# shihchinw/rlShaders

Hardware: AMD Instinct MI355X
Metric: BSDF Gsamples/sec (eval+sample+pdf) (higher is better)
Workload: dtype f32

## Files before the change

__graft_entry__.py:

```python
from __future__ import annotations

import os
import subprocess
import sys
from pathlib import Path

ROOT = Path(__file__).resolve().parent
REF_SRC_DEFAULT = "/root/reference"
for p in (str(ROOT), str(ROOT / "tests")):
    if p not in sys.path:
        sys.path.insert(0, p)


def build() -> None:
    from rlshaders_amd import build as b
    lib = b.build_library(verbose=False)
    assert lib.exists(), lib
    b.build_host_examples()
    b.build_trace_example()
    p = subprocess.run(["make", "-C", str(ROOT / "oracle")], capture_output=True, text=True)
    if p.returncode != 0:
        raise RuntimeError(f"oracle build failed:\n{p.stdout}\n{p.stderr}")
    ref_src = Path(os.environ.get("RLS_REF_SRC", REF_SRC_DEFAULT))
    if (ref_src / "src" / "rlGgx.h").exists():
        p = subprocess.run(["make", "-C", str(ROOT / "oracle"), "ref", f"REF_SRC={ref_src}"], capture_output=True,
                           text=True)
        if p.returncode != 0:
            raise RuntimeError(f"reference build failed:\n{p.stdout}\n{p.stderr}")
    import rlshaders_amd
    rlshaders_amd.load()
    from rlshaders_amd import trace
    trace.load()


def smoke() -> None:
    import numpy as np
    import torch

    import cases
    import oracle_lib as O
    import rlshaders_amd as R
    from gpu_util import dev, ggx_oracle, ggx_sampler, host

    assert torch.cuda.is_available(), "smoke() needs a GPU"
    ctx = R.Context(0)
    n = 1 << 14
    c = cases.ggx_mixed(cases.SEED_PARITY, n)
    x = cases.xi(cases.SEED_PARITY, n, 4)
    s = ggx_sampler(ctx, c)
    out = [host(t) for t in s.reflectRefract(dev(x[0]), dev(x[1]), dev(x[2]), dev(x[3]))]
    ref = ggx_oracle(O, c).reflect_refract(x[0], x[1], x[2], x[3])
    names = ("wi", "f", "pdf", "fresnel", "wt", "weight")
    for name, a, b in zip(names, out, ref):
        st = cases.summarize(cases.rel_err(a, b))
        print(f"smoke {name}: median {st['median']:.2e} p99.9 {st['p999']:.2e} frac>1e-5 {st['frac_gt_1e5']:.2e}")
        assert st["nonfinite"] == 0 and st["max"] <= 1e-5, (name, st)
    f = host(s.evalBrdf(dev(ref[0])))
    assert cases.summarize(cases.rel_err(f, ref[1]))["max"] <= 1e-5
    ctx.close()
    print("smoke ok")


if __name__ == "__main__":
    build()
    if len(sys.argv) > 1 and sys.argv[1] == "smoke":
        smoke()
```

rlshaders_amd/build.py:

```python
from __future__ import annotations

import os
import shutil
import subprocess
import sys
from concurrent.futures import ThreadPoolExecutor
from pathlib import Path

PKG = Path(__file__).resolve().parent
CSRC = PKG / "csrc"
LIBDIR = PKG / "lib"
OBJDIR = PKG / "build"
LIB = LIBDIR / "librlshaders_amd.so"
ARCH = "gfx950"

SOURCES = ["shade.hip", "integrate.hip", "lights.hip", "scatter.hip", "skin.hip", "ggx.hip", "disney.hip", "sss.hip", "alternates.hip", "context.hip", "pipeline.hip",
           "libm_check.hip"]
FAST_UNITS = {"ggx.hip", "disney.hip", "sss.hip", "skin.hip", "integrate.hip", "lights.hip", "scatter.hip", "shade.hip", "alternates.hip"}
HEADERS = [CSRC / "rls_device.hpp", CSRC / "rls_libm.hpp", CSRC / "rls_libm_tables.inc", CSRC / "rls_libm_flavour_args.inc", CSRC / "rls_internal.hpp", CSRC / "rls_loops.hpp",
           PKG.parent / "include" / "rlshaders_amd.h", PKG.parent / "include" / "rlshaders_amd_diag.h"]

HIPCC_FLAGS = [
    f"--offload-arch={ARCH}", "-O3", "-std=c++17", "-fPIC",
    "-ffp-contract=off", "-fno-fast-math",
    "-fno-slp-vectorize",
    "-fno-gpu-rdc",
    "-Wall", "-Wno-unused-function",
]


def _hipcc() -> str:
    exe = shutil.which("hipcc") or "/opt/rocm/bin/hipcc"
    if not os.path.exists(exe):
        raise RuntimeError("hipcc not found: the rlshaders_amd HIP library cannot be built")
    return exe


def _stale(target: Path, deps) -> bool:
    if not target.exists():
        return True
    t = target.stat().st_mtime
    return any(Path(d).stat().st_mtime > t for d in deps)


def sources():
    return [CSRC / s for s in SOURCES if (CSRC / s).exists()]


def build_library(force: bool = False, verbose: bool = False, variant: str = "", defines=(), extra=()) -> Path:
    hipcc = _hipcc()
    LIBDIR.mkdir(exist_ok=True)
    objdir = OBJDIR if not variant else PKG / f"build_{variant}"
    lib = LIB if not variant else LIBDIR / f"librlshaders_amd_{variant}.so"
    objdir.mkdir(exist_ok=True)
    srcs = sources()
    jobs = []
    objs = []
    for src in srcs:
        flavours = [("", "RLS_FAST=0")] + ([("_fast", "RLS_FAST=1")] if src.name in FAST_UNITS else [])
        for suffix, flag in flavours:
            obj = objdir / (src.stem + suffix + ".o")
            objs.append(obj)
            if force or _stale(obj, [src, *HEADERS, Path(__file__)]):
                jobs.append([hipcc, *HIPCC_FLAGS, *extra, f"-cuid=rlshaders_amd.{src.stem}{suffix}", f"-D{flag}",
                             *[f"-D{d}" for d in defines], "-c", str(src), "-o", str(obj)])

    def run(cmd):
        if verbose:
            print(" ".join(cmd), flush=True)
        p = subprocess.run(cmd, capture_output=True, text=True)
        if p.returncode != 0:
            raise RuntimeError(f"hipcc failed:\n{' '.join(cmd)}\n{p.stdout}\n{p.stderr}")
        return p

    if jobs:
        with ThreadPoolExecutor(max_workers=min(4, len(jobs))) as ex:
            list(ex.map(run, jobs))
    if force or jobs or _stale(lib, objs):
        run([hipcc, f"--offload-arch={ARCH}", "-shared", "-fPIC", "-o", str(lib), *map(str, objs)])
    return lib


TRACE_CSRC = PKG / "csrc_trace"
TRACE_SOURCES = ["trace.hip"]
TRACE_LIB = LIBDIR / "librls_trace.so"
TRACE_HEADERS = [TRACE_CSRC / "rls_trace_device.hpp", PKG.parent / "include" / "rlshaders_amd_trace.h"]


def build_trace_library(force: bool = False, verbose: bool = False) -> Path:
    hipcc = _hipcc()
    main = build_library(verbose=verbose)
    objdir = OBJDIR / "trace"
    objdir.mkdir(parents=True, exist_ok=True)
    jobs, objs = [], []
    for name in TRACE_SOURCES:
        src = TRACE_CSRC / name
        for suffix, flag in (("", "RLS_FAST=0"), ("_fast", "RLS_FAST=1")):
            obj = objdir / (src.stem + suffix + ".o")
            objs.append(obj)
            if force or _stale(obj, [src, *HEADERS, *TRACE_HEADERS, Path(__file__)]):
                jobs.append([hipcc, *HIPCC_FLAGS, f"-cuid=rls_trace.{src.stem}{suffix}", f"-D{flag}", "-c", str(src),
                             "-o", str(obj)])

    def run(cmd):
        if verbose:
            print(" ".join(cmd), flush=True)
        p = subprocess.run(cmd, capture_output=True, text=True)
        if p.returncode != 0:
            raise RuntimeError(f"hipcc failed:\n{' '.join(cmd)}\n{p.stdout}\n{p.stderr}")

    if jobs:
        with ThreadPoolExecutor(max_workers=min(4, len(jobs))) as ex:
            list(ex.map(run, jobs))
    if force or jobs or _stale(TRACE_LIB, [*objs, main]):
        run([hipcc, f"--offload-arch={ARCH}", "-shared", "-fPIC", "-o", str(TRACE_LIB), *map(str, objs),
             f"-L{LIBDIR}", "-lrlshaders_amd", "-Wl,-rpath,$ORIGIN"])
    return TRACE_LIB


def build_trace_example(verbose: bool = False) -> Path:
    OBJDIR.mkdir(exist_ok=True)
    lib = build_trace_library(verbose=verbose)
    src, out = PKG / "host" / "example_trace.cpp", OBJDIR / "example_trace"
    if _stale(out, [src, PKG / "host" / "rls_trace.hpp", lib, LIB, *HEADERS, *TRACE_HEADERS]):
        cmd = ["g++", "-std=c++14", "-O2", "-Wall", f"-I{PKG.parent / 'include'}", f"-I{PKG / 'host'}", str(src), "-o", str(out),
               f"-L{LIBDIR}", "-lrls_trace", "-lrlshaders_amd", f"-Wl,-rpath,{LIBDIR}", "-L/opt/rocm/lib", "-Wl,-rpath,/opt/rocm/lib"]
        if verbose:
            print(" ".join(cmd), flush=True)
        p = subprocess.run(cmd, capture_output=True, text=True)
        if p.returncode != 0:
            raise RuntimeError(f"host example example_trace failed to build:\n{p.stdout}\n{p.stderr}")
    return out


def build_host_examples(verbose: bool = False) -> Path:
    OBJDIR.mkdir(exist_ok=True)
    first = OBJDIR / "example_arnold_stub"
    for name in ("example_arnold_stub", "example_multi_gpu", "example_host_pipeline", "test_arnold_stub"):
        src = PKG / "host" / f"{name}.cpp"
        out = OBJDIR / name
        if not src.exists():
            continue
        if _stale(out, [src, PKG / "host" / "rls_batch.hpp", PKG / "host" / "rl_arnold_stub.hpp", LIB, *HEADERS]):
            cmd = ["g++", "-std=c++14", "-O2", "-Wall", "-pthread", f"-I{PKG.parent / 'include'}", f"-I{PKG / 'host'}",
                   str(src), "-o", str(out), f"-L{LIBDIR}", "-lrlshaders_amd", f"-Wl,-rpath,{LIBDIR}",
                   "-L/opt/rocm/lib", "-Wl,-rpath,/opt/rocm/lib"]
            if verbose:
                print(" ".join(cmd), flush=True)
            p = subprocess.run(cmd, capture_output=True, text=True)
            if p.returncode != 0:
                raise RuntimeError(f"host example {name} failed to build:\n{p.stdout}\n{p.stderr}")
    return first


if __name__ == "__main__":
    args = sys.argv[1:]
    variant = args[args.index("--variant") + 1] if "--variant" in args else ""
    defines = [a[2:] for a in args if a.startswith("-D")]
    extra = []
    for i, a in enumerate(args):
        if a.startswith(("-f", "-m", "-O")):
            extra.append(a)
            if a == "-mllvm":
                extra.append(args[i + 1])
    print(build_library(force="--force" in args, verbose=True, variant=variant, defines=defines, extra=extra))
```

rlshaders_amd/csrc/ggx.hip:

```cpp
#include "rls_internal.hpp"

using namespace rlsd;

namespace {

using namespace rlsh;

#define RLS_GGX_ARGS(a0) reload_args(a0)

enum { MIXED = 0, STREAMED_ALL = 1, UNIFORM_MATERIAL = 2 };

template <int MODE>
__device__ __forceinline__ Ggx load_closure(const rls_ggx_closure &c, Idx i, const GgxMaterial &um)
{
    constexpr bool STREAMED = MODE == STREAMED_ALL;
    V3 wo = ld3(c.wo, i), N = ld3(c.N, i), T = ld3(c.T, i);
    const PIndex<Idx> k = pindex<MODE == MIXED>(c.materials, i);
    float kr, kg, kb;
    ldrgb<STREAMED>(c.KsColor, k, kr, kg, kb);
    if (MODE == UNIFORM_MATERIAL)
        return ggx_from_material(um, wo, N, T, c.exiting ? (c.exiting[i.full()] != 0) : false, kr, kg, kb);
    float rough = ldp<STREAMED>(c.specularRoughness, k);
    float ior = ldp<STREAMED>(c.ior, k);
    float aniso = ldp<STREAMED>(c.anisotropic, k);
    bool exiting = c.exiting ? (c.exiting[i.full()] != 0) : false;
    return ggx_make(wo, N, T, exiting, kr, kg, kb, ior, rough, aniso);
}

#ifndef RLS_GGX_WAVES
#define RLS_GGX_WAVES(OP) ((OP) == OP_EVAL ? 6 : 8)
#endif
#define RLS_GGX_ATTR(OP) __launch_bounds__(rlsh::kBlock) __attribute__((amdgpu_waves_per_eu(RLS_GGX_WAVES(OP), RLS_GGX_WAVES(OP))))
template <int OP, int FAST_MATH, int MODE>
__device__ __forceinline__ void ggx_body(const GgxIO &a0)
{
    if (OP == OP_SAMPLE || OP == OP_FUSED || OP == OP_REFLECT_REFRACT || OP == OP_REFRACT || OP == OP_MICROFACET)
        stage_libm_tables();
    GgxMaterial um = {};
    if (MODE == UNIFORM_MATERIAL) {
        const rls_ggx_closure &c = a0.c;
        um = ggx_material_wave_uniform(ggx_material(c.ior.u, c.specularRoughness.u, c.anisotropic.u));
    }
    const TileRange tiles = tile_range(a0.n);
    for (int64_t base = tiles.first; base < tiles.end; base += tiles.step) {
        const Idx i = make_idx(base);
        if (i.full() >= a0.n) continue;
        const GgxIO a = RLS_GGX_ARGS(a0);
        Ggx g = load_closure<MODE>(a.c, i, um);

        if (OP == OP_SAMPLE || OP == OP_FUSED || OP == OP_REFLECT_REFRACT) {
            float rx = ldg(a.rx, i), ry = ldg(a.ry, i);
            VndfView w = vndf_view(g.view, g.fr, g.ax, g.ay);
            V3 M, M2;
            if (OP == OP_REFLECT_REFRACT) {
                float rx2 = ldg(a.rx2, i), ry2 = ldg(a.ry2, i);
                vndf_microfacet_pair(w, g.fr, rx, ry, w, g.fr, rx2, ry2, M, M2);
            } else {
                M = vndf_microfacet(w, g.fr, rx, ry);
            }
            V3 L = reflect_direction(g.view, M);
            float F = ggx_fresnel(g, L, M);
            {
                const GgxIO b = RLS_GGX_ARGS(a0);
                st3(b.wi, i, L);
                if (b.fresnel) stg(b.fresnel, i, F);
            }
            if (OP != OP_SAMPLE) {
                float fr, fg, fb, pdf;
                ggx_eval_pdf<true, true>(g, L, fr, fg, fb, pdf);
                const GgxIO b = RLS_GGX_ARGS(a0);
                strgb(b.f, i, fr, fg, fb);
                stg(b.pdf, i, pdf);
            }
            if (OP == OP_REFLECT_REFRACT) {
                V3 dir;
                ggx_refract(g, M2, dir);
                const float wgt = ggx_sample_weight(g, g.view, dir, M2);
                const GgxIO b = RLS_GGX_ARGS(a0);
                st3(b.wt, i, dir);
                stg(b.weight, i, wgt);
            }
        } else if (OP == OP_EVAL) {
            float fr, fg, fb;
            ggx_eval(g, ld3(a.cwi, i), fr, fg, fb);
            strgb(a.f, i, fr, fg, fb);
        } else if (OP == OP_PDF) {
            stg(a.pdf, i, ggx_pdf(g, ld3(a.cwi, i)));
        } else if (OP == OP_REFRACT) {
            float rx = ldg(a.rx, i), ry = ldg(a.ry, i);
            VndfView w = vndf_view(g.view, g.fr, g.ax, g.ay);
            V3 M = vndf_microfacet(w, g.fr, rx, ry);
            V3 dir;
            bool ok = ggx_refract(g, M, dir);
            st3(a.wt, i, dir);
            stg(a.weight, i, ggx_sample_weight(g, g.view, dir, M));
            if (a.refracted) a.refracted[i.full()] = ok ? 1 : 0;
        } else if (OP == OP_MICROFACET) {
            float rx = ldg(a.rx, i), ry = ldg(a.ry, i);
            V3 M;
            if (a.kernel == RLS_KERNEL_NDF) {
                M = ndf_microfacet(g, rx, ry);
            } else {
                VndfView w = vndf_view(g.view, g.fr, g.ax, g.ay);
                M = vndf_microfacet(w, g.fr, rx, ry);
            }
            st3(a.wi, i, M);
        } else if (OP == OP_NDF_PDF) {
            V3 H = normalize(g.view + ld3(a.cwi, i));
            stg(a.pdf, i, ndf_pdf(g, g.view, H));
        }
    }
}

template <int OP, int FAST_MATH, int MODE>
__global__ RLS_GGX_ATTR(OP) void ggx_kernel(GgxIO a0)
{
    ggx_body<OP, FAST_MATH, MODE>(a0);
}

#if RLS_DIAGNOSTICS
template <int OP, int FAST_MATH, int MODE>
__global__ RLS_GGX_ATTR(OP) void ggx_kernel_stamped(GgxIO a0, unsigned long long *stamps)
{
    ClockStamp<1> cs;
    cs.begin();
    ggx_body<OP, FAST_MATH, MODE>(a0);
    cs.end(stamps);
}
#endif

template <int OP>
rls_status launch_kernel(rls_context *ctx, const GgxIO &io, const char *name)
{
    const rls_ggx_closure &c = io.c;
    const bool streamed = !c.materials.id && c.KsColor.r && c.specularRoughness.v && c.ior.v && c.anisotropic.v;
    const bool uniform = !c.materials.id && !c.specularRoughness.v && !c.ior.v && !c.anisotropic.v;
    if constexpr (OP == OP_REFLECT_REFRACT)
        RLS_STAMPED_LAUNCH(streamed, (ggx_kernel_stamped<OP, RLS_FAST, STREAMED_ALL>),
                           rlsh::grid_for(ctx, io.n, rlsh::kBlock, RLS_CAP_MULT), io, name);
    if (streamed)
        hipLaunchKernelGGL((ggx_kernel<OP, RLS_FAST, STREAMED_ALL>), rlsh::grid_for(ctx, io.n, rlsh::kBlock, RLS_CAP_MULT), dim3(rlsh::kBlock), 0, ctx->stream, io);
    else if (uniform)
        hipLaunchKernelGGL((ggx_kernel<OP, RLS_FAST, UNIFORM_MATERIAL>), rlsh::grid_for_hoisting(ctx, io.n), dim3(rlsh::kBlock), 0, ctx->stream, io);
    else
        hipLaunchKernelGGL((ggx_kernel<OP, RLS_FAST, MIXED>), rlsh::grid_for(ctx, io.n, rlsh::kBlock, RLS_CAP_MULT), dim3(rlsh::kBlock), 0, ctx->stream, io);
    return rlsh::check_launch(name, RLS_FAST);
}

rls_status launch_ggx(rls_context *ctx, int op, const GgxIO &io, const char *name)
{
    switch (op) {
    case OP_SAMPLE: return launch_kernel<OP_SAMPLE>(ctx, io, name);
    case OP_EVAL: return launch_kernel<OP_EVAL>(ctx, io, name);
    case OP_PDF: return launch_kernel<OP_PDF>(ctx, io, name);
    case OP_FUSED: return launch_kernel<OP_FUSED>(ctx, io, name);
    case OP_REFRACT: return launch_kernel<OP_REFRACT>(ctx, io, name);
    case OP_REFLECT_REFRACT: return launch_kernel<OP_REFLECT_REFRACT>(ctx, io, name);
    case OP_MICROFACET: return launch_kernel<OP_MICROFACET>(ctx, io, name);
    default: return launch_kernel<OP_NDF_PDF>(ctx, io, name);
    }
}

}

RLS_FLAVOURS(ggx, rlsh::GgxIO)

#if !RLS_FAST

extern "C" {

rls_status rls_ggx_sample(rls_context *ctx, int64_t n, const rls_ggx_closure *c,
                          const float *rx, const float *ry, rls_vec3 wi, float *fresnel)
{
    RLS_PROLOGUE();
    if (rls_status s = rlsh::check_closure(__func__, c)) return s;
    RLS_REQUIRE(rx && ry, "rx/ry is NULL");
    RLS_REQUIRE(rlsh::has3(wi), "wi plane is NULL");
    GgxIO io = {};
    io.c = *c; io.rx = rx; io.ry = ry; io.wi = wi; io.fresnel = fresnel; io.n = n;
    return dispatch_ggx(ctx, OP_SAMPLE, io, "rls_ggx_sample");
}

rls_status rls_ggx_eval(rls_context *ctx, int64_t n, const rls_ggx_closure *c, rls_cvec3 wi, rls_rgb f)
{
    RLS_PROLOGUE();
    if (rls_status s = rlsh::check_closure(__func__, c)) return s;
    RLS_REQUIRE(rlsh::has3(wi) && rlsh::has3(f), "wi/f plane is NULL");
    GgxIO io = {};
    io.c = *c; io.cwi = wi; io.f = f; io.n = n;
    return dispatch_ggx(ctx, OP_EVAL, io, "rls_ggx_eval");
}

rls_status rls_ggx_pdf(rls_context *ctx, int64_t n, const rls_ggx_closure *c, rls_cvec3 wi, float *pdf)
{
    RLS_PROLOGUE();
    if (rls_status s = rlsh::check_closure(__func__, c)) return s;
    RLS_REQUIRE(rlsh::has3(wi) && pdf, "wi/pdf is NULL");
    GgxIO io = {};
    io.c = *c; io.cwi = wi; io.pdf = pdf; io.n = n;
    return dispatch_ggx(ctx, OP_PDF, io, "rls_ggx_pdf");
}

rls_status rls_ggx_sample_eval_pdf(rls_context *ctx, int64_t n, const rls_ggx_closure *c,
                                   const float *rx, const float *ry,
                                   rls_vec3 wi, rls_rgb f, float *pdf, float *fresnel)
{
    RLS_PROLOGUE();
    if (rls_status s = rlsh::check_closure(__func__, c)) return s;
    RLS_REQUIRE(rx && ry, "rx/ry is NULL");
    RLS_REQUIRE(rlsh::has3(wi) && rlsh::has3(f) && pdf, "wi/f/pdf is NULL");
    GgxIO io = {};
    io.c = *c; io.rx = rx; io.ry = ry; io.wi = wi; io.f = f; io.pdf = pdf; io.fresnel = fresnel; io.n = n;
    return dispatch_ggx(ctx, OP_FUSED, io, "rls_ggx_sample_eval_pdf");
}

rls_status rls_ggx_refract_sample(rls_context *ctx, int64_t n, const rls_ggx_closure *c,
                                  const float *rx, const float *ry,
                                  rls_vec3 wt, float *weight, uint8_t *refracted)
{
    RLS_PROLOGUE();
    if (rls_status s = rlsh::check_closure(__func__, c)) return s;
    RLS_REQUIRE(rx && ry, "rx/ry is NULL");
    RLS_REQUIRE(rlsh::has3(wt) && weight, "wt/weight is NULL");
    GgxIO io = {};
    io.c = *c; io.rx = rx; io.ry = ry; io.wt = wt; io.weight = weight; io.refracted = refracted; io.n = n;
    return dispatch_ggx(ctx, OP_REFRACT, io, "rls_ggx_refract_sample");
}

rls_status rls_ggx_reflect_refract(rls_context *ctx, int64_t n, const rls_ggx_closure *c,
                                   const float *rx, const float *ry, const float *rx2, const float *ry2,
                                   rls_vec3 wi, rls_rgb f, float *pdf, float *fresnel,
                                   rls_vec3 wt, float *weight)
{
    RLS_PROLOGUE();
    if (rls_status s = rlsh::check_closure(__func__, c)) return s;
    RLS_REQUIRE(rx && ry && rx2 && ry2, "random-number plane is NULL");
    RLS_REQUIRE(rlsh::has3(wi) && rlsh::has3(f) && pdf, "wi/f/pdf is NULL");
    RLS_REQUIRE(rlsh::has3(wt) && weight, "wt/weight is NULL");
    GgxIO io = {};
    io.c = *c; io.rx = rx; io.ry = ry; io.rx2 = rx2; io.ry2 = ry2;
    io.wi = wi; io.f = f; io.pdf = pdf; io.fresnel = fresnel; io.wt = wt; io.weight = weight; io.n = n;
    return dispatch_ggx(ctx, OP_REFLECT_REFRACT, io, "rls_ggx_reflect_refract");
}

rls_status rls_ggx_microfacet(rls_context *ctx, int64_t n, const rls_ggx_closure *c, int kernel,
                              const float *rx, const float *ry, rls_vec3 m)
{
    RLS_PROLOGUE();
    if (rls_status s = rlsh::check_closure(__func__, c)) return s;
    RLS_REQUIRE(kernel == RLS_KERNEL_VNDF || kernel == RLS_KERNEL_NDF, "unknown sampling kernel");
    RLS_REQUIRE(rx && ry, "rx/ry is NULL");
    RLS_REQUIRE(rlsh::has3(m), "m plane is NULL");
    GgxIO io = {};
    io.c = *c; io.rx = rx; io.ry = ry; io.wi = m; io.kernel = kernel; io.n = n;
    return dispatch_ggx(ctx, OP_MICROFACET, io, "rls_ggx_microfacet");
}

rls_status rls_ggx_ndf_pdf(rls_context *ctx, int64_t n, const rls_ggx_closure *c, rls_cvec3 wi, float *pdf)
{
    RLS_PROLOGUE();
    if (rls_status s = rlsh::check_closure(__func__, c)) return s;
    RLS_REQUIRE(rlsh::has3(wi) && pdf, "wi/pdf is NULL");
    GgxIO io = {};
    io.c = *c; io.cwi = wi; io.pdf = pdf; io.n = n;
    return dispatch_ggx(ctx, OP_NDF_PDF, io, "rls_ggx_ndf_pdf");
}

}

#endif
```

rlshaders_amd/csrc/rls_libm.hpp:

```cpp
#pragma once

#include <math.h>
#include <stdint.h>
#include <string.h>

#if defined(__HIPCC__)
#include <hip/hip_runtime.h>
#define RLM_FN __host__ __device__ __forceinline__
#else
#define RLM_FN static inline
#endif

namespace rlm {

RLM_FN uint32_t f2u(float x)
{
#if defined(__HIP_DEVICE_COMPILE__)
    return __float_as_uint(x);
#else
    uint32_t u; memcpy(&u, &x, 4); return u;
#endif
}
RLM_FN float u2f(uint32_t u)
{
#if defined(__HIP_DEVICE_COMPILE__)
    return __uint_as_float(u);
#else
    float x; memcpy(&x, &u, 4); return x;
#endif
}
RLM_FN float fabs32(float x) { return u2f(f2u(x) & 0x7fffffffu); }

RLM_FN float div32(float a, float b) { return a / b; }

#ifndef RLM_GLIBC_FMA
#define RLM_GLIBC_FMA 1
#endif
RLM_FN double mad(double a, double b, double c)
{
#if RLM_GLIBC_FMA
    return __builtin_fma(a, b, c);
#else
    return a * b + c;
#endif
}

template <bool GUARDED = true>
RLM_FN float sqrt32(float x)
{
#if defined(__HIP_DEVICE_COMPILE__)
    if (GUARDED && __builtin_expect((f2u(x) & 0x7fffffffu) - 1u < 0x0f800000u - 1u, 0)) return sqrtf(x);
    float s = __builtin_amdgcn_sqrtf(x);
    const float sm = __uint_as_float(__float_as_uint(s) - 1u);
    const float sp = __uint_as_float(__float_as_uint(s) + 1u);
    const float rm = __builtin_fmaf(-sm, s, x);
    const float rp = __builtin_fmaf(-sp, s, x);
    s = (0.0f >= rm) ? sm : s;
    s = (0.0f < rp) ? sp : s;
    return s;
#else
    return sqrtf(x);
#endif
}
RLM_FN float sqrt32_1p(float y) { return sqrt32<false>(1.0f + y); }
RLM_FN float sqrt32_1m(float t) { return sqrt32<false>(1.0f - t); }

RLM_FN float rcp32_w(float x)
{
#if defined(__HIP_DEVICE_COMPILE__)
    float r = __builtin_amdgcn_rcpf(x);
    const float e = __builtin_fmaf(-x, r, 1.0f);
    r = __builtin_fmaf(e, r, r);
    return __builtin_amdgcn_div_fixupf(r, x, 1.0f);
#else
    return 1.0f / x;
#endif
}
RLM_FN float rcp32(float x)
{
#if defined(__HIP_DEVICE_COMPILE__)
    if (__builtin_expect(__builtin_amdgcn_classf(x, 0x90) || __builtin_fabsf(x) > 0x1p126f, 0)) return 1.0f / x;
    return rcp32_w(x);
#else
    return 1.0f / x;
#endif
}

RLM_FN float div32_m(float a, float b)
{
#if defined(__HIP_DEVICE_COMPILE__)
    float y = __builtin_amdgcn_rcpf(b);
    const float e = __builtin_fmaf(-b, y, 1.0f);
    y = __builtin_fmaf(e, y, y);
    const float q0 = a * y;
    const float r = __builtin_fmaf(-b, q0, a);
    return __builtin_fmaf(r, y, q0);
#else
    return a / b;
#endif
}

RLM_FN float div32_const_w(float x, float c, float rc)
{
#if defined(__HIP_DEVICE_COMPILE__)
    const float q0 = x * rc;
    const float r = __builtin_fmaf(-c, q0, x);
    return __builtin_fmaf(r, rc, q0);
#else
    (void)rc;
    return x / c;
#endif
}
RLM_FN float div32_const(float x, float c, float rc)
{
#if defined(__HIP_DEVICE_COMPILE__)
    if (__builtin_expect(!(__builtin_fabsf(x) >= 0x1p-100f && __builtin_fabsf(x) <= 0x1p100f), 0)) return x / c;
    const float q0 = x * rc;
    const float r = __builtin_fmaf(-c, q0, x);
    return __builtin_fmaf(r, rc, q0);
#else
    (void)rc;
    return x / c;
#endif
}

RLM_FN float rcp32_hi(float x)
{
#if defined(__HIP_DEVICE_COMPILE__)
    if (__builtin_expect(!(__builtin_fabsf(x) <= 0x1p126f), 0)) return 1.0f / x;
    return rcp32_w(x);
#else
    return 1.0f / x;
#endif
}

RLM_FN float atan32(float x)
{
    const float atanhi0 = u2f(0x3eed6338u), atanhi1 = u2f(0x3f490fdau), atanhi2 = u2f(0x3f7b985eu),
                atanhi3 = u2f(0x3fc90fdau);
    const float atanlo0 = u2f(0x31ac3769u), atanlo1 = u2f(0x33222168u), atanlo2 = u2f(0x33140fb4u),
                atanlo3 = u2f(0x33a22168u);
    const float aT0 = u2f(0x3eaaaaabu), aT1 = u2f(0xbe4ccccdu), aT2 = u2f(0x3e124925u), aT3 = u2f(0xbde38e38u),
                aT4 = u2f(0x3dba2e6eu), aT5 = u2f(0xbd9d8795u), aT6 = u2f(0x3d886b35u), aT7 = u2f(0xbd6ef16bu),
                aT8 = u2f(0x3d4bda59u), aT9 = u2f(0xbd15a221u), aT10 = u2f(0x3c8569d7u);
    const int32_t hx = (int32_t)f2u(x);
    const int32_t ix = hx & 0x7fffffff;
    if (ix >= 0x4c000000) {
        if (ix > 0x7f800000) return x + x;
        return hx > 0 ? atanhi3 + atanlo3 : -atanhi3 - atanlo3;
    }
    int id;
    float hi = 0.0f, lo = 0.0f;
    if (ix < 0x3ee00000) {
        if (ix < 0x31000000) return x;
        id = -1;
    } else {
        x = fabs32(x);
        if (ix < 0x3f980000) {
            if (ix < 0x3f300000) {
                id = 0; hi = atanhi0; lo = atanlo0;
                x = (2.0f * x - 1.0f) / (2.0f + x);
            } else {
                id = 1; hi = atanhi1; lo = atanlo1;
                x = (x - 1.0f) / (x + 1.0f);
            }
        } else {
            if (ix < 0x401c0000) {
                id = 2; hi = atanhi2; lo = atanlo2;
                x = (x - 1.5f) / (1.0f + 1.5f * x);
            } else {
                id = 3; hi = atanhi3; lo = atanlo3;
                x = -1.0f / x;
            }
        }
    }
    const float z = x * x;
    const float w = z * z;
    const float s1 = z * (aT0 + w * (aT2 + w * (aT4 + w * (aT6 + w * (aT8 + w * aT10)))));
    const float s2 = w * (aT1 + w * (aT3 + w * (aT5 + w * (aT7 + w * aT9))));
    if (id < 0) return x - x * (s1 + s2);
    const float r = hi - ((x * (s1 + s2) - lo) - x);
    return hx < 0 ? -r : r;
}

RLM_FN float atan2_32(float y, float x)
{
    const float tiny = 1.0e-30f;
    const float pi_o_4 = u2f(0x3f490fdbu), pi_o_2 = u2f(0x3fc90fdbu), pi = u2f(0x40490fdbu), pi_lo = u2f(0xb3bbbd2eu);
    const int32_t hx = (int32_t)f2u(x), hy = (int32_t)f2u(y);
    const int32_t ix = hx & 0x7fffffff, iy = hy & 0x7fffffff;
    if (ix > 0x7f800000 || iy > 0x7f800000) return x + y;
    if (hx == 0x3f800000) return atan32(y);
    const int m = ((hy >> 31) & 1) | ((hx >> 30) & 2);
    if (iy == 0) {
        switch (m) {
        case 0:
        case 1: return y;
        case 2: return pi + tiny;
        default: return -pi - tiny;
        }
    }
    if (ix == 0) return hy < 0 ? -pi_o_2 - tiny : pi_o_2 + tiny;
    if (ix == 0x7f800000) {
        if (iy == 0x7f800000) {
            switch (m) {
            case 0: return pi_o_4 + tiny;
            case 1: return -pi_o_4 - tiny;
            case 2: return 3.0f * pi_o_4 + tiny;
            default: return -3.0f * pi_o_4 - tiny;
            }
        }
        switch (m) {
        case 0: return 0.0f;
        case 1: return -0.0f;
        case 2: return pi + tiny;
        default: return -pi - tiny;
        }
    }
    if (iy == 0x7f800000) return hy < 0 ? -pi_o_2 - tiny : pi_o_2 + tiny;
    const int32_t k = (iy - ix) >> 23;
    float z;
    if (k > 60) z = pi_o_2 + 0.5f * pi_lo;
    else if (hx < 0 && k < -60) z = 0.0f;
    else z = atan32(fabs32(y / x));
    switch (m) {
    case 0: return z;
    case 1: return u2f(f2u(z) ^ 0x80000000u);
    case 2: return pi - (z - pi_lo);
    default: return (z - pi_lo) - pi;
    }
}

RLM_FN float acos32(float x)
{
    const float pi = u2f(0x40490fdau), pio2_hi = u2f(0x3fc90fdau), pio2_lo = u2f(0x33a22168u);
    const float pS0 = u2f(0x3e2aaaabu), pS1 = u2f(0xbea6b090u), pS2 = u2f(0x3e4e0aa8u), pS3 = u2f(0xbd241146u),
                pS4 = u2f(0x3a4f7f04u), pS5 = u2f(0x3811ef08u);
    const float qS1 = u2f(0xc019d139u), qS2 = u2f(0x4001572du), qS3 = u2f(0xbf303361u), qS4 = u2f(0x3d9dc62eu);
    const int32_t hx = (int32_t)f2u(x);
    const int32_t ix = hx & 0x7fffffff;
    if (ix == 0x3f800000) return hx > 0 ? 0.0f : pi + 2.0f * pio2_lo;
    if (ix > 0x3f800000) return (x - x) / (x - x);
    if (ix < 0x3f000000) {
        if (ix <= 0x23000000) return pio2_hi + pio2_lo;
        const float z = x * x;
        const float p = z * (pS0 + z * (pS1 + z * (pS2 + z * (pS3 + z * (pS4 + z * pS5)))));
        const float q = 1.0f + z * (qS1 + z * (qS2 + z * (qS3 + z * qS4)));
        const float r = p / q;
        return pio2_hi - (x - (pio2_lo - x * r));
    }
    if (hx < 0) {
        const float z = (1.0f + x) * 0.5f;
        const float p = z * (pS0 + z * (pS1 + z * (pS2 + z * (pS3 + z * (pS4 + z * pS5)))));
        const float q = 1.0f + z * (qS1 + z * (qS2 + z * (qS3 + z * qS4)));
        const float s = sqrt32(z);
        const float r = p / q;
        const float w = r * s - pio2_lo;
        return pi - 2.0f * (s + w);
    }
    const float z = (1.0f - x) * 0.5f;
    const float s = sqrt32(z);
    const float df = u2f(f2u(s) & 0xfffff000u);
    const float c = (z - df * df) / (s + df);
    const float p = z * (pS0 + z * (pS1 + z * (pS2 + z * (pS3 + z * (pS4 + z * pS5)))));
    const float q = 1.0f + z * (qS1 + z * (qS2 + z * (qS3 + z * qS4)));
    const float r = p / q;
    const float w = r * s + c;
    return 2.0f * (df + w);
}

RLM_FN float kernel_tan32(float x, float y, int iy)
{
    const float pio4 = u2f(0x3f490fdau), pio4lo = u2f(0x33222168u);
    const float T0 = u2f(0x3eaaaaabu), T1 = u2f(0x3e088889u), T2 = u2f(0x3d5d0dd1u), T3 = u2f(0x3cb327a4u),
                T4 = u2f(0x3c11371fu), T5 = u2f(0x3b6b6916u), T6 = u2f(0x3abede48u), T7 = u2f(0x3a1a26c8u),
                T8 = u2f(0x398137b9u), T9 = u2f(0x38a3f445u), T10 = u2f(0x3895c07au), T11 = u2f(0xb79bae5fu),
                T12 = u2f(0x37d95384u);
    const int32_t hx = (int32_t)f2u(x);
    const int32_t ix = hx & 0x7fffffff;
    if (ix < 0x39000000) {
        if ((int)x == 0) {
            if ((ix | (iy + 1)) == 0) return 1.0f / fabs32(x);
            if (iy == 1) return x;
            return -1.0f / x;
        }
    }
    if (ix >= 0x3f2ca140) {
        if (hx < 0) { x = -x; y = -y; }
        const float zz = pio4 - x;
        const float ww = pio4lo - y;
        x = zz + ww;
        y = 0.0f;
        if (fabs32(x) < 0x1p-13f) return (float)(1 - ((hx >> 30) & 2)) * (float)iy * (1.0f - 2.0f * (float)iy * x);
    }
    float z = x * x;
    float w = z * z;
    float r = T1 + w * (T3 + w * (T5 + w * (T7 + w * (T9 + w * T11))));
    float v = z * (T2 + w * (T4 + w * (T6 + w * (T8 + w * (T10 + w * T12)))));
    float s = z * x;
    r = y + z * (s * (r + v) + y);
    r += T0 * s;
    w = x + r;
    if (ix >= 0x3f2ca140) {
        v = (float)iy;
        return (float)(1 - ((hx >> 30) & 2)) * (v - 2.0f * (x - (w * w / (w + v) - r)));
    }
    if (iy == 1) return w;
    z = u2f(f2u(w) & 0xfffff000u);
    v = r - (z - x);
    const float a = -1.0f / w;
    const float t = u2f(f2u(a) & 0xfffff000u);
    s = 1.0f + t * z;
    return t + a * (s + t * v);
}


RLM_FN double reduce_large(uint32_t xi, int *np)
{
    static const uint32_t inv_pio4[24] = {
        0xa2u, 0xa2f9u, 0xa2f983u, 0xa2f9836eu, 0xf9836e4eu, 0x836e4e44u, 0x6e4e4415u, 0x4e441529u,
        0x441529fcu, 0x1529fc27u, 0x29fc2757u, 0xfc2757d1u, 0x2757d1f5u, 0x57d1f534u, 0xd1f534ddu, 0xf534ddc0u,
        0x34ddc0dbu, 0xddc0db62u, 0xc0db6295u, 0xdb629599u, 0x6295993cu, 0x95993c43u, 0x993c4390u, 0x3c439041u };
    const double pi63 = 0x1.921FB54442D18p-62;
    const uint32_t *arr = &inv_pio4[(xi >> 26) & 15];
    const int shift = (int)(xi >> 23) & 7;
    xi = (xi & 0xffffffu) | 0x800000u;
    xi <<= shift;
    uint64_t res0 = (uint64_t)(uint32_t)(xi * arr[0]);
    const uint64_t res1 = (uint64_t)xi * arr[4];
    const uint64_t res2 = (uint64_t)xi * arr[8];
    res0 = (res2 >> 32) | (res0 << 32);
    res0 += res1;
    const uint64_t n = (res0 + (1ULL << 61)) >> 62;
    res0 -= n << 62;
    *np = (int)n;
    return (double)(int64_t)res0 * pi63;
}

RLM_FN void sincos32(float y, float *sinp, float *cosp)
{
    const double hpi_inv = 0x1.45F306DC9C883p+23;
    const double hpi = 0x1.921FB54442D18p0;
    const double C0 = 0x1p0, C1 = -0x1.ffffffd0c621cp-2, C2 = 0x1.55553e1068f19p-5, C3 = -0x1.6c087e89a359dp-10,
                 C4 = 0x1.99343027bf8c3p-16;
    const double S1 = -0x1.555545995a603p-3, S2 = 0x1.1107605230bc4p-7, S3 = -0x1.994eb3774cf24p-13;
    const uint32_t top = (f2u(y) >> 20) & 0x7ffu;
    double x = (double)y;
    int n = 0, m = 0;
    bool tiny = false;
    if (top < 0x3f4u) {
        tiny = top < 0x398u;
    } else if (top < 0x42fu) {
        const double r = x * hpi_inv;
        n = ((int32_t)r + 0x800000) >> 24;
// ... 610 lines not shown
```

Before: 68.46.

## Route streamed GGX reflect/refract through a separately built companion kernel library

Adds a separately compiled ggx2 library holding a specialised reflect/refract kernel. It precomputes reciprocals of roughness alphas and |vn| once per sample, so divisions in D and the pdf become multiplies when a wave-wide ballot shows every lane's operands are in range. It also uses a single-compare sqrt guard and forces a waves_per_eu occupancy attribute. The non-fast library locates the companion via dladdr/dlopen and uses it for streamed inputs unless RLS_GGX2=0. This adds a runtime dynamic-loading dependency and a second build, and risks ulp differences in the reciprocal path.

```diff
diff --git a/__graft_entry__.py b/__graft_entry__.py
--- a/__graft_entry__.py
+++ b/__graft_entry__.py
@@ -16,6 +16,7 @@
     from rlshaders_amd import build as b
     lib = b.build_library(verbose=False)
     assert lib.exists(), lib
+    assert b.build_ggx2_library().exists()
     b.build_host_examples()
     b.build_trace_example()
     p = subprocess.run(["make", "-C", str(ROOT / "oracle")], capture_output=True, text=True)
diff --git a/rlshaders_amd/build.py b/rlshaders_amd/build.py
--- a/rlshaders_amd/build.py
+++ b/rlshaders_amd/build.py
@@ -118,6 +118,30 @@
     return TRACE_LIB
 
 
+GGX2_CSRC = PKG / "csrc_ggx2"
+GGX2_LIB = LIBDIR / "librls_ggx2.so"
+GGX2_HEADERS = [GGX2_CSRC / "rls_ggx2.h"]
+
+
+def build_ggx2_library(force: bool = False, verbose: bool = False, out: Path = None, defines=()) -> Path:
+    hipcc = _hipcc()
+    LIBDIR.mkdir(exist_ok=True)
+    objdir = OBJDIR / "ggx2"
+    objdir.mkdir(parents=True, exist_ok=True)
+    src = GGX2_CSRC / "ggx2.hip"
+    lib = Path(out) if out else GGX2_LIB
+    obj = objdir / ("ggx2.o" if not out else f"ggx2_{lib.parent.name}.o")
+    if out or force or _stale(obj, [src, *HEADERS, *GGX2_HEADERS, Path(__file__)]) or _stale(lib, [obj]):
+        for cmd in ([hipcc, *HIPCC_FLAGS, "-cuid=rls_ggx2.ggx2", "-DRLS_FAST=0", *[f"-D{d}" for d in defines], "-c", str(src), "-o", str(obj)],
+                    [hipcc, f"--offload-arch={ARCH}", "-shared", "-fPIC", "-o", str(lib), str(obj)]):
+            if verbose:
+                print(" ".join(cmd), flush=True)
+            p = subprocess.run(cmd, capture_output=True, text=True)
+            if p.returncode != 0:
+                raise RuntimeError(f"hipcc failed:\n{' '.join(cmd)}\n{p.stdout}\n{p.stderr}")
+    return lib
+
+
 def build_trace_example(verbose: bool = False) -> Path:
     OBJDIR.mkdir(exist_ok=True)
     lib = build_trace_library(verbose=verbose)
diff --git a/rlshaders_amd/csrc/ggx.hip b/rlshaders_amd/csrc/ggx.hip
--- a/rlshaders_amd/csrc/ggx.hip
+++ b/rlshaders_amd/csrc/ggx.hip
@@ -1,4 +1,11 @@
 #include "rls_internal.hpp"
+
+#if !RLS_FAST
+#include <dlfcn.h>
+#include <string.h>
+#include <string>
+#include "../csrc_ggx2/rls_ggx2.h"
+#endif
 
 using namespace rlsd;
 
@@ -129,6 +136,29 @@
 }
 #endif
 
+#if !RLS_FAST
+typedef int (*Ggx2Launch)(const void *io, unsigned grid, void *stream);
+static Ggx2Launch ggx2_lookup()
+{
+    const char *e = getenv("RLS_GGX2");
+    if (e && e[0] == '0' && e[1] == 0) return nullptr;
+    Dl_info self;
+    if (!dladdr(reinterpret_cast<const void *>(&ggx2_lookup), &self) || !self.dli_fname) return nullptr;
+    const char *slash = strrchr(self.dli_fname, '/');
+    if (!slash) return nullptr;
+    std::string path(self.dli_fname, (size_t)(slash - self.dli_fname) + 1);
+    path += RLS_GGX2_LIBRARY;
+    void *h = dlopen(path.c_str(), RTLD_NOW | RTLD_LOCAL);
+    if (!h) return nullptr;
+    return reinterpret_cast<Ggx2Launch>(dlsym(h, "rls_ggx2_launch_reflect_refract"));
+}
+static Ggx2Launch ggx2_launch()
+{
+    static const Ggx2Launch f = ggx2_lookup();
+    return f;
+}
+#endif
+
 template <int OP>
 rls_status launch_kernel(rls_context *ctx, const GgxIO &io, const char *name)
 {
@@ -138,6 +168,16 @@
     if constexpr (OP == OP_REFLECT_REFRACT)
         RLS_STAMPED_LAUNCH(streamed, (ggx_kernel_stamped<OP, RLS_FAST, STREAMED_ALL>),
                            rlsh::grid_for(ctx, io.n, rlsh::kBlock, RLS_CAP_MULT), io, name);
+#if !RLS_FAST
+    if constexpr (OP == OP_REFLECT_REFRACT) {
+        if (streamed) {
+            if (const Ggx2Launch companion = ggx2_launch()) {
+                companion(&io, rlsh::grid_for(ctx, io.n, rlsh::kBlock, RLS_CAP_MULT).x, ctx->stream);
+                return rlsh::check_launch(name, RLS_FAST);
+            }
+        }
+    }
+#endif
     if (streamed)
         hipLaunchKernelGGL((ggx_kernel<OP, RLS_FAST, STREAMED_ALL>), rlsh::grid_for(ctx, io.n, rlsh::kBlock, RLS_CAP_MULT), dim3(rlsh::kBlock), 0, ctx->stream, io);
     else if (uniform)
diff --git a/rlshaders_amd/csrc/rls_libm.hpp b/rlshaders_amd/csrc/rls_libm.hpp
--- a/rlshaders_amd/csrc/rls_libm.hpp
+++ b/rlshaders_amd/csrc/rls_libm.hpp
@@ -45,11 +45,18 @@
 #endif
 }
 
+#ifndef RLM_SQRT_GUARD_ONE_COMPARE
+#define RLM_SQRT_GUARD_ONE_COMPARE 0
+#endif
 template <bool GUARDED = true>
 RLM_FN float sqrt32(float x)
 {
 #if defined(__HIP_DEVICE_COMPILE__)
+#if RLM_SQRT_GUARD_ONE_COMPARE
+    if (GUARDED && __builtin_expect(!(__builtin_fabsf(x) >= 0x1p-96f), 0)) return sqrtf(x);
+#else
     if (GUARDED && __builtin_expect((f2u(x) & 0x7fffffffu) - 1u < 0x0f800000u - 1u, 0)) return sqrtf(x);
+#endif
     float s = __builtin_amdgcn_sqrtf(x);
     const float sm = __uint_as_float(__float_as_uint(s) - 1u);
     const float sp = __uint_as_float(__float_as_uint(s) + 1u);
diff --git a/rlshaders_amd/csrc_ggx2/ggx2.hip b/rlshaders_amd/csrc_ggx2/ggx2.hip
--- /dev/null
+++ b/rlshaders_amd/csrc_ggx2/ggx2.hip
@@ -0,0 +1,150 @@
+#ifndef RLS_GGX2_SQRT_GUARD
+#define RLS_GGX2_SQRT_GUARD 1
+#endif
+#ifndef RLS_GGX2_RECIPS
+#define RLS_GGX2_RECIPS 1
+#endif
+#define RLM_SQRT_GUARD_ONE_COMPARE RLS_GGX2_SQRT_GUARD
+#include "../csrc/rls_internal.hpp"
+
+#include "rls_ggx2.h"
+
+using namespace rlsd;
+
+namespace {
+
+using namespace rlsh;
+
+enum { STREAMED_ALL = 1 };
+
+struct GgxRecips { float yax, yay, yvn; };
+
+RLS_DEV GgxRecips ggx2_recips(const Ggx &g)
+{
+    GgxRecips y;
+    const bool win = g.ax <= 0x1p14f && g.ay <= 0x1p14f;
+    y.yax = win ? rlm::rcp32_w(g.ax) : 0.0f;
+    y.yay = win ? rlm::rcp32_w(g.ay) : 0.0f;
+    const float avn = absf(g.vn);
+    y.yvn = (avn >= 0x1p-14f && avn <= 0x1p14f) ? rlm::rcp32_w(avn) : 0.0f;
+    return y;
+}
+
+RLS_DEV float ggx2_D(const Ggx &g, const GgxRecips &y, V3 m)
+{
+    float mu = dot(m, g.fr.U);
+    float mv = dot(m, g.fr.V);
+    float mn2 = sqr(dot(g.fr.N, m));
+    const float amu = absf(mu), amv = absf(mv);
+    const bool plain = !(amu <= 0x1p40f && amv <= 0x1p40f && amu >= 0x1p-75f && amv >= 0x1p-75f) || y.yax == 0.0f;
+    float qu, qv;
+    if (!RLS_GGX2_RECIPS || __builtin_expect(__builtin_amdgcn_ballot_w64(plain) != 0ull, 0)) {
+        qu = R_DIVH(mu, g.ax);
+        qv = R_DIVH(mv, g.ay);
+    } else {
+        qu = rlm::div32_y(mu, g.ax, y.yax);
+        qv = rlm::div32_y(mv, g.ay, y.yay);
+    }
+    float den = g.ax * g.ay * sqr(sqr(qu) + sqr(qv) + mn2);
+    return R_DIV(kInvPi, den);
+}
+
+RLS_DEV void ggx2_eval_pdf(const Ggx &g, const GgxRecips &y, V3 L, float &fr, float &fg, float &fb, float &pdf)
+{
+    V3 H = normalize_h(L + g.view);
+    float d = ggx2_D(g, y, H);
+    {
+        const float num = d * ggx_G1_view(g, H);
+        const bool plain = !(absf(num) <= 0x1p40f) || y.yvn == 0.0f;
+        float p;
+        if (!RLS_GGX2_RECIPS || __builtin_expect(__builtin_amdgcn_ballot_w64(plain) != 0ull, 0)) p = R_DIV(num, absf(g.vn)) * 0.25f;
+        else p = rlm::div32_y(num, absf(g.vn), y.yvn) * 0.25f;
+        pdf = maxf(p, kEps);
+    }
+    bool small = absf(g.ksR) < kEps && absf(g.ksG) < kEps && absf(g.ksB) < kEps;
+    if (is_zero(L) || small) {
+        fr = 0.0f; fg = 0.0f; fb = 0.0f;
+        return;
+    }
+    V3 hr = H * sgnf(g.vn);
+    float rw = ggx_fresnel(g, g.view, hr);
+    float ln = absf(dot(L, g.fr.N));
+    float vn = absf(g.vn);
+    float refl = R_DIV(rw * ggx_G(g, L, hr) * d * 0.25f, ln * vn);
+    float lns = dot(L, g.fr.N);
+    fr = g.ksR * refl * lns;
+    fg = g.ksG * refl * lns;
+    fb = g.ksB * refl * lns;
+}
+
+RLS_DEV Ggx load_closure(const rls_ggx_closure &c, Idx i)
+{
+    V3 wo = ld3(c.wo, i), N = ld3(c.N, i), T = ld3(c.T, i);
+    const PIndex<Idx> k = pindex<false>(c.materials, i);
+    float kr, kg, kb;
+    ldrgb<true>(c.KsColor, k, kr, kg, kb);
+    float rough = ldp<true>(c.specularRoughness, k);
+    float ior = ldp<true>(c.ior, k);
+    float aniso = ldp<true>(c.anisotropic, k);
+    bool exiting = c.exiting ? (c.exiting[i.full()] != 0) : false;
+    return ggx_make(wo, N, T, exiting, kr, kg, kb, ior, rough, aniso);
+}
+
+template <int OP, int FAST_MATH, int MODE>
+__global__ __launch_bounds__(rlsh::kBlock) __attribute__((amdgpu_waves_per_eu(8, 8))) void ggx_kernel(GgxIO a0)
+{
+    static_assert(OP == OP_REFLECT_REFRACT && FAST_MATH == 0 && MODE == STREAMED_ALL, "one instantiation");
+    stage_libm_tables();
+    const TileRange tiles = tile_range(a0.n);
+    for (int64_t base = tiles.first; base < tiles.end; base += tiles.step) {
+        const Idx i = make_idx(base);
+        if (i.full() >= a0.n) continue;
+        const GgxIO a = reload_args(a0);
+        Ggx g = load_closure(a.c, i);
+        const GgxRecips y = ggx2_recips(g);
+
+        float rx = ldg(a.rx, i), ry = ldg(a.ry, i);
+        VndfView w = vndf_view(g.view, g.fr, g.ax, g.ay);
+        V3 M, M2;
+        float rx2 = ldg(a.rx2, i), ry2 = ldg(a.ry2, i);
+        vndf_microfacet_pair(w, g.fr, rx, ry, w, g.fr, rx2, ry2, M, M2);
+        V3 L = reflect_direction(g.view, M);
+        float F = ggx_fresnel(g, L, M);
+        {
+            const GgxIO b = reload_args(a0);
+            st3(b.wi, i, L);
+            if (b.fresnel) stg(b.fresnel, i, F);
+        }
+        {
+            float fr, fg, fb, pdf;
+            ggx2_eval_pdf(g, y, L, fr, fg, fb, pdf);
+            const GgxIO b = reload_args(a0);
+            strgb(b.f, i, fr, fg, fb);
+            stg(b.pdf, i, pdf);
+        }
+        {
+            V3 dir;
+            ggx_refract(g, M2, dir);
+            const float wgt = ggx_sample_weight(g, g.view, dir, M2);
+            const GgxIO b = reload_args(a0);
+            st3(b.wt, i, dir);
+            stg(b.weight, i, wgt);
+        }
+    }
+}
+
+}
+
+extern "C" {
+
+int rls_ggx2_launch_reflect_refract(const void *io, unsigned grid, void *stream)
+{
+    const GgxIO &a = *static_cast<const GgxIO *>(io);
+    hipLaunchKernelGGL((ggx_kernel<OP_REFLECT_REFRACT, 0, STREAMED_ALL>), dim3(grid), dim3(rlsh::kBlock), 0,
+                       static_cast<hipStream_t>(stream), a);
+    return 0;
+}
+
+const char *rls_ggx2_code_id(void) { return RLS_GGX2_REVISION; }
+
+}
diff --git a/rlshaders_amd/csrc_ggx2/rls_ggx2.h b/rlshaders_amd/csrc_ggx2/rls_ggx2.h
--- /dev/null
+++ b/rlshaders_amd/csrc_ggx2/rls_ggx2.h
@@ -0,0 +1,13 @@
+#pragma once
+
+#define RLS_GGX2_LIBRARY "librls_ggx2.so"
+#define RLS_GGX2_REVISION "ggx2-r07.1"
+
+#ifdef __cplusplus
+extern "C" {
+#endif
+int rls_ggx2_launch_reflect_refract(const void *io, unsigned grid, void *stream);
+const char *rls_ggx2_code_id(void);
+#ifdef __cplusplus
+}
+#endif
```

Measured after the change: 69.15, median of 6. Within noise of the previous version (+1.0%).
